# tangjiapeng/DiffuScene

Measured on AMD Instinct MI355X. Metric: denoiser steps/sec (train + 1000-step sample) at B=256, N=80 objects, higher is better.
Workload: dtype f32 (operands split 3xbf16, 6 products, f32 accumulate); 1 GPU; uncond living/dining rooms (config/uncond/diffusion_livingrooms_instancond_lat32_v.yaml scaled to N=80), B=256 scenes per GPU, N=80, C=65, T=1000, mode=both; global_batch=256, parallelism=single

## Files before the change

diffuscene_amd/_lib.py:

```python
import ctypes as C
import os

_HERE = os.path.dirname(os.path.abspath(__file__))
LIB_PATH = os.path.join(_HERE, "libdiffuscene_hip.so")
if os.environ.get("DSC_HIP_LIB"):
    LIB_PATH = os.path.abspath(os.environ["DSC_HIP_LIB"])

ACT_NONE, ACT_GELU, ACT_SILU, ACT_LEAKY01 = 0, 1, 2, 3
SS_NONE, SS_PER_TOKEN, SS_PER_SCENE, SS_PER_SLOT, SS_BY_INDEX = 0, 1, 2, 3, 4
MEAN_EPS, MEAN_X0, MEAN_V = 0, 1, 2
TILE_GN_80_W8, TILE_GN_80_W4, TILE_160x256, TILE_160x128_W4 = 1, 2, 5, 8
TILE_WAVE_GN, TILE_WAVE_DENSE, TILE_WAVE_GN_64 = 10, 11, 12
F32_TILE_160x256, F32_TILE_160x128, F32_TILE_128x128, F32_TILE_96x128, F32_TILE_64x64 = 0, 1, 2, 3, 4
DSC_PLANES_NONE = -100
GEMM_ROW_INVARIANT = 1
WS_MAX = 64
MAX_TOKENS_PER_SCENE = 160
STATS_MAX_OBJECTS, STATS_ONE_WAVE_MAX = 160, 32

_ERR = {-1: "DSC_EINVAL (bad shape / null pointer)", -2: "DSC_EALIGN (16-byte alignment required)",
        -3: "DSC_ERANGE (size outside kernel limits)"}

c_f32p = C.c_void_p
c_i64p = C.c_void_p
# ... 115 lines not shown
    "dsc_knn_cov_f32": (C.c_int, [c_f32p, C.c_int64, C.c_void_p, C.c_int32, C.c_int32, c_f32p, C.c_int64, C.c_void_p]),
    "dsc_gather_max_f32": (C.c_int, [c_f32p, C.c_int64, C.c_void_p, C.c_int32, C.c_int32, C.c_int32, c_f32p, C.c_int64,
                                     C.c_void_p, C.c_void_p]),
    "dsc_gather_max_bwd_f32": (C.c_int, [c_f32p, C.c_int64, C.c_void_p, C.c_void_p, C.c_int32, C.c_int32, C.c_int32, c_f32p,
                                         C.c_int64, C.c_void_p]),
    "dsc_bn_workspace_floats": (C.c_int64, [C.c_int64, C.c_int32]),
    "dsc_batchnorm_fwd_f32": (C.c_int, [c_f32p, C.c_int64, c_f32p, c_f32p, C.c_int64, C.c_int32, C.c_float, C.c_float,
                                        C.c_int32, c_f32p, c_f32p, c_f32p, c_f32p, c_f32p, c_f32p, c_f32p, C.c_int64,
                                        C.c_void_p]),
    "dsc_batchnorm_eval_f32": (C.c_int, [c_f32p, C.c_int64, c_f32p, c_f32p, c_f32p, c_f32p, C.c_int64, C.c_int32, C.c_int32,
                                         c_f32p, C.c_void_p]),
    "dsc_batchnorm_bwd_f32": (C.c_int, [c_f32p, c_f32p, c_f32p, c_f32p, c_f32p, C.c_int64, C.c_int32, C.c_int32, c_f32p,
                                        c_f32p, c_f32p, c_f32p, C.c_int64, C.c_void_p]),
    "dsc_rowmax_f32": (C.c_int, [c_f32p, C.c_int64, C.c_int32, C.c_int32, C.c_int32, c_f32p, C.c_void_p, C.c_void_p]),
    "dsc_rowmax_bwd_f32": (C.c_int, [c_f32p, C.c_void_p, C.c_int32, C.c_int32, C.c_int32, c_f32p, C.c_void_p]),
    "dsc_point_affine_f32": (C.c_int, [c_f32p, C.c_int64, C.c_int32, c_f32p, C.c_int64, c_f32p, C.c_int32, C.c_int32,
                                       C.c_int32, C.c_int32, c_f32p, C.c_void_p]),
    "dsc_point_affine_bwd_f32": (C.c_int, [c_f32p, c_f32p, C.c_int64, C.c_int32, c_f32p, C.c_int64, C.c_int32, C.c_int32,
                                           C.c_int32, C.c_int32, c_f32p, C.c_int64, c_f32p, C.c_int64, c_f32p, c_f32p,
                                           C.c_int64, C.c_void_p]),
    "dsc_postfilter_compact_f32": (C.c_int, [c_f32p, C.c_int32, C.c_int32, C.c_int32, C.c_int32, C.c_int32, C.c_int32, c_f32p,
                                             C.c_void_p, C.c_void_p]),
    "dsc_gemm_tn_f32": (C.c_int, [c_f32p, C.c_int64, C.c_int32, c_f32p, C.c_int64, C.c_int32, c_f32p, C.c_int64, c_f32p,
                                  C.c_int64, c_f32p, C.c_int32, C.c_int32, C.c_int32, c_f32p, C.c_int64, C.c_void_p]),
    "dsc_gemm_tn_workspace_floats": (C.c_int64, [C.c_int32, C.c_int32, C.c_int32]),
    "dsc_gemm_tn_grouped_f32": (C.c_int, [C.c_void_p, C.c_int32, C.c_int32, C.c_int32, c_f32p, C.c_int64, C.c_int64,
                                          C.c_void_p]),
    "dsc_gemm_tn_grouped_split_f32": (C.c_int, [C.c_void_p, C.c_int32, C.c_int32, C.c_void_p, C.c_int32, C.c_int32, c_f32p, C.c_int64,
                                                C.c_int64, C.c_int32, C.c_void_p]),
    "dsc_set_tn_split_form": (C.c_int, [C.c_int32]),
    "dsc_get_tn_split_form": (C.c_int, []),
    "dsc_colsum_f32": (C.c_int, [c_f32p, C.c_int64, C.c_int32, C.c_int32, c_f32p, c_f32p, C.c_int64, C.c_void_p]),
    "dsc_colsum_grouped_f32": (C.c_int, [C.c_void_p, C.c_int32, C.c_int32, C.c_void_p]),
    "dsc_gn_silu_bwd_f32": (C.c_int, [c_f32p, C.c_int64, c_f32p, C.c_int64, c_f32p, c_f32p, c_f32p, C.c_int64, C.c_int32,
                                      c_f32p, C.c_int64, c_f32p, c_f32p, c_f32p, C.c_int64, c_f32p, C.c_int64, C.c_int32,
                                      C.c_int32, C.c_int32, C.c_float, C.c_void_p]),
    "dsc_weight_standardize_bwd_f32": (C.c_int, [C.POINTER(WsBwdItem), C.c_int32, C.c_float, C.c_void_p]),
    "dsc_layernorm_bwd_f32": (C.c_int, [c_f32p, C.c_int64, c_f32p, c_f32p, C.c_int64, c_f32p, C.c_int64, c_f32p, C.c_int64, c_f32p,
                                        C.c_int32, C.c_int32, C.c_int32, C.c_float, C.c_void_p]),
    "dsc_linear_attention_bwd_f32": (C.c_int, [c_f32p, C.c_int64] * 7 + [C.c_int32, C.c_int32, C.c_int32, C.c_float,
                                                                          C.c_void_p]),
    "dsc_attention_bwd_f32": (C.c_int, [c_f32p, C.c_int64] * 7 + [C.c_int32, C.c_int32, C.c_float, C.c_void_p]),
    "dsc_retrieve_nearest_f32": (C.c_int, [c_f32p, C.c_void_p, C.c_void_p, c_f32p, C.c_void_p, C.c_void_p, C.c_int32,
                                           C.c_int32, C.c_int32, C.c_void_p, c_f32p, C.c_void_p]),
    "dsc_box_bounds_f32": (C.c_int, [c_f32p, c_f32p, c_f32p, C.c_void_p, C.c_int32, C.c_int32, c_f32p, C.c_void_p]),
    "dsc_scene_stats_f32": (C.c_int, [c_f32p, c_f32p, C.c_void_p, C.c_void_p, C.c_int32, C.c_int32, C.c_int32, C.c_int32,
                                      C.c_void_p, C.c_void_p, C.c_void_p, C.c_void_p, C.c_void_p, C.c_void_p, c_f32p, C.c_void_p]),
    "dsc_encode_scene_batch_f32": (C.c_int, [c_i64p, c_f32p, c_f32p, c_f32p, c_f32p, c_f32p, C.c_int32, C.c_int32, c_i64p,
                                             C.c_void_p, C.c_void_p, C.c_void_p, C.c_int32, C.POINTER(C.c_double), c_f32p,
                                             C.c_int64, c_i64p, C.c_int32, C.c_int32, C.c_void_p]),
    "dsc_chamfer3d_forward_f32": (C.c_int, [c_f32p, c_f32p, c_f32p, c_f32p, C.c_void_p, C.c_void_p, C.c_int32, C.c_int32,
                                            C.c_int32, C.c_void_p]),
    "dsc_chamfer3d_backward_f32": (C.c_int, [c_f32p, c_f32p, c_f32p, c_f32p, C.c_void_p, C.c_void_p, c_f32p, c_f32p,
                                             C.c_int32, C.c_int32, C.c_int32, C.c_void_p]),
    "dsc_grad_sumsq_f32": (C.c_int, [C.c_void_p, C.c_int32, C.c_void_p, C.c_void_p]),
    "dsc_clip_coef_f32": (C.c_int, [C.c_void_p, C.c_int32, C.c_float, c_f32p, c_f32p, C.c_void_p]),
    "dsc_adam_step_f32": (C.c_int, [C.c_void_p, C.c_int32, C.c_float, C.c_float, C.c_float, C.c_float, C.c_float, C.c_float,
                                    c_f32p, C.c_void_p]),
    "dsc_adam_ema_step_f32": (C.c_int, [C.c_void_p, C.c_void_p, C.c_int32, C.c_float, C.c_float, C.c_float, C.c_float, C.c_float,
                                        C.c_float, c_f32p, C.c_float, C.c_void_p]),
    "dsc_ema_update_f32": (C.c_int, [C.c_void_p, C.c_void_p, C.c_int32, C.c_float, C.c_void_p]),
    "dsc_ema_swap_f32": (C.c_int, [C.c_void_p, C.c_void_p, C.c_int32, C.c_void_p]),
    "dsc_ddpm_loss_f32": (C.c_int, [c_f32p, c_f32p, c_f32p, c_i64p, c_f32p, c_f32p, c_f32p, c_f32p, C.POINTER(C.c_float),
                                    c_f32p, c_f32p, c_f32p] + [C.c_int32] * 12 + [C.c_float, C.c_int32, C.c_void_p]),
    "dsc_copy2d_f32": (C.c_int, [c_f32p, C.c_int64, c_f32p, C.c_int64, C.c_int32, C.c_int32, C.c_void_p]),
    "dsc_add2d_f32": (C.c_int, [c_f32p, C.c_int64, c_f32p, C.c_int64, C.c_int32, C.c_int32, C.c_void_p]),
# ... 45 lines not shown
    "dsc_avgpool_rows_bwd_f32": (C.c_int, [c_f32p, c_f32p] + [C.c_int32] * 3 + [C.c_void_p]),
}

_lib = None


class HipLibraryMissing(RuntimeError):
    pass


def load():
    global _lib
    if _lib is not None:
        return _lib
    if not os.path.exists(LIB_PATH):
        raise HipLibraryMissing(
            "%s not found: build it with `python __graft_entry__.py` (hipcc --offload-arch=gfx950). "
            "diffuscene_amd has no CPU or PyTorch fallback." % LIB_PATH)
    import torch
    lib = C.CDLL(LIB_PATH)
    for name, (res, args) in SIGNATURES.items():
        try:
            fn = getattr(lib, name)
        except AttributeError as e:
            raise HipLibraryMissing("symbol %s missing from %s" % (name, LIB_PATH)) from e
        fn.restype = res
        fn.argtypes = args
    if lib.dsc_get_gemm_arithmetic() < 0:
        raise ValueError("DSC_GEMM=%r: must be 'split' (default) or 'f32'" % os.environ.get("DSC_GEMM"))
    if lib.dsc_get_tn_split_form() < 0:
        raise ValueError("DSC_TN_FORM=%r: must be '2' (default), '1' or '0'" % os.environ.get("DSC_TN_FORM"))
    if lib.dsc_get_split_wave() < 0:
        raise ValueError("DSC_WAVE=%r: must be '1' / 'auto' (default) or '0'" % os.environ.get("DSC_WAVE"))
    _lib = lib
    return lib


def split_enabled():
    return load().dsc_get_gemm_arithmetic() == 1


def gemm_mode():
    lib = load()
    if lib.dsc_get_gemm_arithmetic() != 1:
        return 0
    return (2 if lib.dsc_get_split_wave() == 1 else 1) + 10 * lib.dsc_get_tn_split_form()


def set_split_wave(on):
    prev = load().dsc_get_split_wave() == 1
    check(load().dsc_set_split_wave(1 if on else 0), "dsc_set_split_wave")
    return prev


def set_gemm_arithmetic(name):
    if name not in ("split", "f32"):
        raise ValueError("gemm arithmetic must be 'split' or 'f32', got %r" % (name,))
    prev = "split" if split_enabled() else "f32"
    check(load().dsc_set_gemm_arithmetic(1 if name == "split" else 0), "dsc_set_gemm_arithmetic")
    return prev


def device_error_count(reset=False):
    n = load().dsc_device_error_count(1 if reset else 0)
    if n < 0:
        raise RuntimeError("dsc_device_error_count failed (HIP error)")
    return int(n)


def check_indices(where):
    if os.environ.get("DSC_CHECK_INDICES", "0") == "1":
        n = device_error_count(reset=True)
        if n:
            raise IndexError("%s: %d out-of-range device timestep(s) were clamped into the schedule tables" % (where, n))


def check(rc, what):
    if rc != 0:
        raise RuntimeError("%s failed: %s" % (what, _ERR.get(rc, "hipError_t %d" % rc)))


def fn(name):
    return getattr(load(), name)
```

diffuscene_amd/csrc/train.hip:

```cpp
#define DSC_BAD_INDEX_COUNTER
#include "dsc_common.h"

namespace {

constexpr int TN_BK = 32;
constexpr int TN_LD = 132;

struct TnArgs {
    const float* a1; long lda1; int k1;
    const float* a2; long lda2; int k2;
    const float* dy; long ldd;
    float* out; long ldo;
    float* bias_out;
    long slab;
    long bias_slab;
    int m, n, kvalid;
    int chunk;
    int ktiles;
};

__device__ __forceinline__ void tn_block(const TnArgs& p, const int it, const int jt, const int split, float* As, float* Bs) {
    const int tid = threadIdx.x, lane = tid & 63, wave = tid >> 6;
    const int wi = wave >> 1, wj = wave & 1;
    const int l31 = lane & 31, half = lane >> 5;
    const int i0 = it * 128, j0 = jt * 128;
    const long m_begin = (long)split * p.chunk;
    const long m_end = (m_begin + p.chunk < p.m) ? m_begin + p.chunk : p.m;

    const float* ab;
    long lda;
    int ic;
    int kseg;
    if (i0 < p.k1) { ab = p.a1; lda = p.lda1; ic = i0; kseg = p.k1; }
// ... 523 lines not shown
            p.dss[(tok0 + j) * p.ld_dss + c] = du * gh;
            p.dss[(tok0 + j) * p.ld_dss + p.C + c] = du;
        }
        zc[j * 64] = xh;
        dc[j * 64] = dxh;
    }
    const float m1 = block_sum(S1, red) * inv_cnt;
    const float m2 = block_sum(S2, red) * inv_cnt;
    float Gz = 0.f;
    {
        float* op = p.dz + (tok0 + tq) * p.lddz + c;
        const long os = 4 * p.lddz;
        for (int j = tq; j < N; j += 4) {
            const float dzv = rs * (dc[j * 64] - m1 - zc[j * 64] * m2);
            *op = dzv;
            op += os;
            Gz += dzv;
        }
    }
    csum[0][tq][cl] = Gg; csum[1][tq][cl] = Gb; csum[2][tq][cl] = Gz; csum[3][tq][cl] = Gsc; csum[4][tq][cl] = Gsh;
    __syncthreads();
    if (tq == 0) {
        const long o = (long)b * p.pstride + c;
        p.dgamma_p[o] = (csum[0][0][cl] + csum[0][1][cl]) + (csum[0][2][cl] + csum[0][3][cl]);
        p.dbeta_p[o] = (csum[1][0][cl] + csum[1][1][cl]) + (csum[1][2][cl] + csum[1][3][cl]);
        p.dbias_p[o] = (csum[2][0][cl] + csum[2][1][cl]) + (csum[2][2][cl] + csum[2][3][cl]);
        if (p.dss && p.ss_mode == DSC_SS_PER_SCENE) {
            p.dss[(long)b * p.ld_dss + c] = (csum[3][0][cl] + csum[3][1][cl]) + (csum[3][2][cl] + csum[3][3][cl]);
            p.dss[(long)b * p.ld_dss + p.C + c] = (csum[4][0][cl] + csum[4][1][cl]) + (csum[4][2][cl] + csum[4][3][cl]);
        }
    }
}

template <int NIT>
__global__ __launch_bounds__(256) void gn_silu_bwd_reg_kernel(const GnBwdArgs p) {
    __shared__ float red[2][4];
    __shared__ float csum[5][4][64];
    const int b = blockIdx.x >> 3, g = blockIdx.x & 7;
    const int cq = threadIdx.x & 15, tr = threadIdx.x >> 4;
    const int wave = threadIdx.x >> 6;
    const int c = g * 64 + cq * 4;
    const int N = p.n_tok;
    const long tok0 = (long)b * N;
    const float inv_cnt = 1.0f / (64.0f * (float)N);
    int phase = 0;
    auto bsum = [&](float v) {
        v = wave_sum(v);
        float* r = red[phase & 1];
        ++phase;
        if ((threadIdx.x & 63) == 0) r[wave] = v;
        __syncthreads();
        return (r[0] + r[1]) + (r[2] + r[3]);
    };
    f32x4 zv[NIT], dv[NIT];
    float s = 0.f;
#pragma unroll
    for (int i = 0; i < NIT; ++i) {
        const int j = tr + 16 * i;
        const bool ok = j < N;
        const long row = tok0 + (ok ? j : 0);
        zv[i] = *reinterpret_cast<const f32x4*>(p.z + row * p.ldz + c);
        dv[i] = *reinterpret_cast<const f32x4*>(p.dy + row * p.ldy + c);
        if (!ok) { zv[i] = f32x4{0.f, 0.f, 0.f, 0.f}; dv[i] = zv[i]; }
        s += (zv[i][0] + zv[i][1]) + (zv[i][2] + zv[i][3]);
    }
    const float mu = bsum(s) * inv_cnt;
    s = 0.f;
#pragma unroll
    for (int i = 0; i < NIT; ++i)
        if (tr + 16 * i < N) {
#pragma unroll
            for (int e = 0; e < 4; ++e) { const float d = zv[i][e] - mu; s += d * d; }
        }
    const float rs = 1.0f / sqrtf(bsum(s) * inv_cnt + p.eps);
    const f32x4 ga = *reinterpret_cast<const f32x4*>(p.gamma + c);
    const f32x4 be = *reinterpret_cast<const f32x4*>(p.beta + c);
    const float* ssb = nullptr;
    long ss_step = 0;
    if (p.ss) {
        if (p.ss_mode == DSC_SS_PER_TOKEN) { ssb = p.ss + tok0 * p.ld_ss; ss_step = p.ld_ss; }
        else if (p.ss_mode == DSC_SS_PER_SCENE) { ssb = p.ss + (long)b * p.ld_ss; ss_step = 0; }
        else if (p.ss_mode == DSC_SS_PER_SLOT) { ssb = p.ss; ss_step = p.ld_ss; }
    }
    const bool dss_rows = p.dss && p.ss_mode != DSC_SS_PER_SCENE && ssb;
    float S1 = 0.f, S2 = 0.f;
    f32x4 Gg = {0.f, 0.f, 0.f, 0.f}, Gb = Gg, Gsc = Gg, Gsh = Gg, Gz = Gg;
#pragma unroll
    for (int i = 0; i < NIT; ++i) {
        const int j = tr + 16 * i;
        if (j < N) {
            f32x4 s1 = {1.f, 1.f, 1.f, 1.f}, sh = {0.f, 0.f, 0.f, 0.f};
            if (ssb) {
                const float* sr = ssb + (long)j * ss_step;
                const f32x4 a = *reinterpret_cast<const f32x4*>(sr + c);
                sh = *reinterpret_cast<const f32x4*>(sr + p.C + c);
#pragma unroll
                for (int e = 0; e < 4; ++e) s1[e] = 1.0f + a[e];
            }
            f32x4 xh, dxh, d_sc, d_sh;
#pragma unroll
            for (int e = 0; e < 4; ++e) {
                xh[e] = (zv[i][e] - mu) * rs;
                const float gh = ga[e] * xh[e] + be[e];
                const float u = gh * s1[e] + sh[e];
                const float sig = __builtin_amdgcn_rcpf(1.0f + __expf(-u));
                const float du = dv[i][e] * (sig * (1.0f + u * (1.0f - sig)));
                const float dgh = du * s1[e];
                dxh[e] = dgh * ga[e];
                S1 += dxh[e]; S2 += dxh[e] * xh[e];
                Gg[e] += dgh * xh[e]; Gb[e] += dgh; Gsc[e] += du * gh; Gsh[e] += du;
                d_sc[e] = du * gh; d_sh[e] = du;
            }
            if (dss_rows) {
                *reinterpret_cast<f32x4*>(p.dss + (tok0 + j) * p.ld_dss + c) = d_sc;
                *reinterpret_cast<f32x4*>(p.dss + (tok0 + j) * p.ld_dss + p.C + c) = d_sh;
            }
            zv[i] = xh;
            dv[i] = dxh;
        }
    }
    const float m1 = bsum(S1) * inv_cnt;
    const float m2 = bsum(S2) * inv_cnt;
#pragma unroll
    for (int i = 0; i < NIT; ++i) {
        const int j = tr + 16 * i;
        if (j < N) {
            f32x4 dzv;
#pragma unroll
            for (int e = 0; e < 4; ++e) { dzv[e] = rs * (dv[i][e] - m1 - zv[i][e] * m2); Gz[e] += dzv[e]; }
            *reinterpret_cast<f32x4*>(p.dz + (tok0 + j) * p.lddz + c) = dzv;
        }
    }
    auto fold = [&](f32x4 v, int slot) {
#pragma unroll
        for (int e = 0; e < 4; ++e) {
            float t = v[e];
            t += __shfl_xor(t, 16, 64);
            t += __shfl_xor(t, 32, 64);
            if ((threadIdx.x & 63) < 16) csum[slot][wave][cq * 4 + e] = t;
        }
    };
    fold(Gg, 0); fold(Gb, 1); fold(Gz, 2); fold(Gsc, 3); fold(Gsh, 4);
    __syncthreads();
    if (threadIdx.x < 64) {
        const int cl = threadIdx.x;
        const long o = (long)b * p.pstride + g * 64 + cl;
        p.dgamma_p[o] = (csum[0][0][cl] + csum[0][1][cl]) + (csum[0][2][cl] + csum[0][3][cl]);
        p.dbeta_p[o] = (csum[1][0][cl] + csum[1][1][cl]) + (csum[1][2][cl] + csum[1][3][cl]);
        p.dbias_p[o] = (csum[2][0][cl] + csum[2][1][cl]) + (csum[2][2][cl] + csum[2][3][cl]);
        if (p.dss && p.ss_mode == DSC_SS_PER_SCENE) {
            p.dss[(long)b * p.ld_dss + g * 64 + cl] = (csum[3][0][cl] + csum[3][1][cl]) + (csum[3][2][cl] + csum[3][3][cl]);
            p.dss[(long)b * p.ld_dss + p.C + g * 64 + cl] = (csum[4][0][cl] + csum[4][1][cl]) + (csum[4][2][cl] + csum[4][3][cl]);
        }
    }
}

struct WsBwdItem { const float* w; const float* dwh; float* dw; int rows; int cols; };
struct WsBwdBatch { WsBwdItem it[DSC_WS_MAX]; };

__global__ __launch_bounds__(256) void ws_bwd_kernel(const WsBwdBatch bch, const float eps) {
    __shared__ float red[4];
    const WsBwdItem it = bch.it[blockIdx.y];
    const int row = blockIdx.x;
    if (row >= it.rows) return;
    const float* w = it.w + (long)row * it.cols;
    const float* g = it.dwh + (long)row * it.cols;
    float* o = it.dw + (long)row * it.cols;
    constexpr int MAXE = 8;
    float v[MAXE], gv[MAXE];
    float s = 0.f;
#pragma unroll
    for (int i = 0; i < MAXE; ++i) {
        const int c = threadIdx.x + 256 * i;
        v[i] = (c < it.cols) ? w[c] : 0.f;
        gv[i] = (c < it.cols) ? g[c] : 0.f;
        s += v[i];
    }
    const float inv = 1.0f / (float)it.cols;
    const float mean = block_sum(s, red) * inv;
    float s2 = 0.f;
#pragma unroll
    for (int i = 0; i < MAXE; ++i) {
        const int c = threadIdx.x + 256 * i;
        const float d = (c < it.cols) ? v[i] - mean : 0.f;
        s2 += d * d;
// ... 641 lines not shown
                              int64_t workspace_floats, dsc_stream_t stream) {
    if (!x || !out || m < 1 || n < 1) return DSC_EINVAL;
    int splits = (m + 255) / 256;
    if (splits > 64) splits = 64;
    const int chunk = (m + splits - 1) / splits;
    splits = (m + chunk - 1) / chunk;
    hipStream_t s = static_cast<hipStream_t>(stream);
    if (splits == 1) {
        DSC_CLEAR_STALE_ERROR();
        hipLaunchKernelGGL(colsum_kernel, dim3((n + 63) / 64, 1), dim3(256), 0, s, x, (long)ldx, m, n, chunk, out);
        DSC_LAUNCH_CHECK();
        return 0;
    }
    if (!workspace || workspace_floats < (int64_t)splits * n) return DSC_EINVAL;
    DSC_CLEAR_STALE_ERROR();
    hipLaunchKernelGGL(colsum_kernel, dim3((n + 63) / 64, splits), dim3(256), 0, s, x, (long)ldx, m, n, chunk, workspace);
    DSC_LAUNCH_CHECK();
    DSC_CLEAR_STALE_ERROR();
    hipLaunchKernelGGL(reduce_slabs_kernel, dim3((n + 255) / 256), dim3(256), 0, s, workspace, (long)n, splits, out, (long)n);
    DSC_LAUNCH_CHECK();
    return 0;
}

extern "C" int dsc_colsum_grouped_f32(const dsc_colsum_item* items_dev, int32_t count, int32_t max_n, dsc_stream_t stream) {
    if (!items_dev || count < 1 || max_n < 1) return DSC_EINVAL;
    static_assert(sizeof(dsc_colsum_item) == sizeof(ColsumItem), "dsc_colsum_item layout");
    DSC_CLEAR_STALE_ERROR();
    hipLaunchKernelGGL(colsum_grouped_kernel, dim3((max_n + 63) / 64, count), dim3(256), 0, static_cast<hipStream_t>(stream),
                       reinterpret_cast<const ColsumItem*>(items_dev));
    DSC_LAUNCH_CHECK();
    return 0;
}

extern "C" int dsc_gn_silu_bwd_f32(const float* z, int64_t ldz, const float* dy, int64_t ldy, const float* gamma,
                                   const float* beta, const float* scale_shift, int64_t ld_ss, int32_t ss_mode,
                                   float* dz, int64_t lddz, float* dgamma_p, float* dbeta_p, float* dbias_p,
                                   int64_t partial_stride, float* dss, int64_t ld_dss, int32_t scenes,
                                   int32_t tokens_per_scene, int32_t channels, float eps, dsc_stream_t stream) {
    if (!z || !dy || !gamma || !beta || !dz || !dgamma_p || !dbeta_p || !dbias_p) return DSC_EINVAL;
    if (scenes < 1 || tokens_per_scene < 1 || channels != 512) return DSC_ERANGE;
    if (ss_mode != DSC_SS_NONE && !scale_shift) return DSC_EINVAL;
    GnBwdArgs p{z, (long)ldz, dy, (long)ldy, gamma, beta, ss_mode != DSC_SS_NONE ? scale_shift : nullptr, (long)ld_ss,
                ss_mode, dz, (long)lddz, dgamma_p, dbeta_p, dbias_p, (long)partial_stride, dss, (long)ld_dss, tokens_per_scene,
                channels, eps};
    if (tokens_per_scene > 160) return DSC_ERANGE;
    const size_t lds = (size_t)2 * tokens_per_scene * 64 * sizeof(float);
    DSC_CLEAR_STALE_ERROR();
    const bool v4 = ((ldz | ldy | lddz) & 3) == 0 && dsc_aligned16(z) && dsc_aligned16(dy) && dsc_aligned16(dz) &&
                    dsc_aligned16(gamma) && dsc_aligned16(beta) &&
                    (!p.ss || (dsc_aligned16(p.ss) && (ld_ss & 3) == 0)) &&
                    (!dss || (dsc_aligned16(dss) && (ld_dss & 3) == 0));
    if (lds > 48 * 1024) {
        static bool raised = false;
        if (!raised) {
            hipError_t e = hipFuncSetAttribute(reinterpret_cast<const void*>(gn_silu_bwd_kernel),
                                               hipFuncAttributeMaxDynamicSharedMemorySize, 96 * 1024);
            if (e != hipSuccess) return (int)e;
            raised = true;
        }
    }
    hipStream_t hs = static_cast<hipStream_t>(stream);
    if (v4 && tokens_per_scene <= 32)
        hipLaunchKernelGGL(gn_silu_bwd_reg_kernel<2>, dim3(scenes * 8), dim3(256), 0, hs, p);
    else if (v4 && tokens_per_scene <= 80)
        hipLaunchKernelGGL(gn_silu_bwd_reg_kernel<5>, dim3(scenes * 8), dim3(256), 0, hs, p);
    else if (v4)
        hipLaunchKernelGGL(gn_silu_bwd_reg_kernel<10>, dim3(scenes * 8), dim3(256), 0, hs, p);
    else
        hipLaunchKernelGGL(gn_silu_bwd_kernel, dim3(scenes * 8), dim3(256), lds, static_cast<hipStream_t>(stream), p);
    DSC_LAUNCH_CHECK();
    return 0;
}

extern "C" int dsc_weight_standardize_bwd_f32(const dsc_ws_bwd_item* items, int32_t count, float eps, dsc_stream_t stream) {
    if (!items || count < 1 || count > DSC_WS_MAX) return DSC_EINVAL;
    WsBwdBatch b;
    int maxrows = 0;
    for (int i = 0; i < count; ++i) {
        if (!items[i].w || !items[i].dw_std || !items[i].dw || items[i].rows < 1 || items[i].cols < 1) return DSC_EINVAL;
        if (items[i].cols > 2048) return DSC_ERANGE;
        b.it[i] = WsBwdItem{items[i].w, items[i].dw_std, items[i].dw, items[i].rows, items[i].cols};
        if (items[i].rows > maxrows) maxrows = items[i].rows;
    }
    DSC_CLEAR_STALE_ERROR();
    hipLaunchKernelGGL(ws_bwd_kernel, dim3(maxrows, count), dim3(256), 0, static_cast<hipStream_t>(stream), b, eps);
    DSC_LAUNCH_CHECK();
    return 0;
}

extern "C" int dsc_layernorm_bwd_f32(const float* x, int64_t ldx, const float* g, const float* dy, int64_t ldy, float* dx,
                                     int64_t lddx, const float* addend, int64_t ldadd, float* dg_partial, int32_t partial_rows,
                                     int32_t m, int32_t d, float eps, dsc_stream_t stream) {
    if (!x || !g || !dy || !dx || !dg_partial || m < 1 || partial_rows < 1) return DSC_EINVAL;
    if (d != 512) return DSC_ERANGE;
    if (!dsc_aligned16(x) || !dsc_aligned16(g) || !dsc_aligned16(dy) || !dsc_aligned16(dx) || (ldx & 3) || (ldy & 3) ||
        (lddx & 3) || (addend && (!dsc_aligned16(addend) || (ldadd & 3)))) return DSC_EALIGN;
    DSC_CLEAR_STALE_ERROR();
    hipLaunchKernelGGL(layernorm_bwd_kernel, dim3(partial_rows), dim3(256), 0, static_cast<hipStream_t>(stream),
                       x, (long)ldx, g, dy, (long)ldy, dx, (long)lddx, addend, (long)ldadd, dg_partial, m, eps);
    DSC_LAUNCH_CHECK();
// ... 392 lines not shown
```

include/diffuscene_hip.h:

```cpp
#ifndef DIFFUSCENE_HIP_H
#define DIFFUSCENE_HIP_H

#include <stdint.h>

#ifdef __cplusplus
extern "C" {
#endif

typedef void* dsc_stream_t;

#define DSC_EINVAL   (-1)
#define DSC_EALIGN   (-2)
#define DSC_ERANGE   (-3)

#define DSC_ACT_NONE 0
#define DSC_ACT_GELU 1
#define DSC_ACT_SILU 2
#define DSC_ACT_LEAKY01 3

#define DSC_SS_NONE      0
#define DSC_SS_PER_TOKEN 1
#define DSC_SS_PER_SCENE 2
#define DSC_SS_PER_SLOT  3
#define DSC_SS_BY_INDEX  4
// ... 256 lines not shown
int64_t dsc_gemm_tn_workspace_floats(int32_t m, int32_t n, int32_t k);

typedef struct dsc_tn_group {
    const float* a1; int64_t lda1; int32_t k1;
    const float* a2; int64_t lda2; int32_t k2;
    const float* dy; int64_t ldd;
    float* out; int64_t ldo;
    float* dbias;
    int32_t m, n, kvalid;
    int32_t tile0;
    int64_t ws_offset;
    int32_t tile0s;
} dsc_tn_group;
int dsc_gemm_tn_grouped_f32(const dsc_tn_group* groups_dev, int32_t count, int32_t total_tiles, int32_t splits,
                            float* workspace, int64_t workspace_floats, int64_t workspace_needed, dsc_stream_t stream);
int dsc_gemm_tn_grouped_split_f32(const dsc_tn_group* groups_dev, int32_t count, int32_t total_tiles, const int32_t* block_map_dev,
                                  int32_t blocks, int32_t splits, float* workspace, int64_t workspace_floats, int64_t workspace_needed,
                                  int32_t tile_k, dsc_stream_t stream);

int dsc_set_tn_split_form(int32_t form);
int dsc_get_tn_split_form(void);

int dsc_colsum_f32(const float* x, int64_t ldx, int32_t m, int32_t n, float* out, float* workspace,
                   int64_t workspace_floats, dsc_stream_t stream);

typedef struct dsc_colsum_item { const float* x; int64_t ldx; int32_t m, n; float* out; } dsc_colsum_item;
int dsc_colsum_grouped_f32(const dsc_colsum_item* items_dev, int32_t count, int32_t max_n, dsc_stream_t stream);

int dsc_gn_silu_bwd_f32(const float* z, int64_t ldz, const float* dy, int64_t ldy, const float* gamma,
                        const float* beta, const float* scale_shift, int64_t ld_ss, int32_t ss_mode,
                        float* dz, int64_t lddz, float* dgamma_p, float* dbeta_p, float* dbias_p, int64_t partial_stride,
                        float* dss, int64_t ld_dss, int32_t scenes, int32_t tokens_per_scene, int32_t channels,
                        float eps, dsc_stream_t stream);

typedef struct dsc_ws_bwd_item { const float* w; const float* dw_std; float* dw; int32_t rows; int32_t cols; } dsc_ws_bwd_item;
int dsc_weight_standardize_bwd_f32(const dsc_ws_bwd_item* items, int32_t count, float eps, dsc_stream_t stream);

int dsc_layernorm_bwd_f32(const float* x, int64_t ldx, const float* g, const float* dy, int64_t ldy, float* dx,
                          int64_t lddx, const float* addend, int64_t ldadd, float* dg_partial, int32_t partial_rows, int32_t m,
                          int32_t d, float eps, dsc_stream_t stream);

int dsc_linear_attention_bwd_f32(const float* q, int64_t ldq, const float* k, int64_t ldk, const float* v, int64_t ldv,
                                 const float* dout, int64_t ldo, float* dq, int64_t lddq, float* dk, int64_t lddk,
                                 float* dv, int64_t lddv, int32_t scenes, int32_t nq, int32_t nk, float scale,
                                 dsc_stream_t stream);

int dsc_attention_bwd_f32(const float* q, int64_t ldq, const float* k, int64_t ldk, const float* v, int64_t ldv,
                          const float* dout, int64_t ldo, float* dq, int64_t lddq, float* dk, int64_t lddk,
                          float* dv, int64_t lddv, int32_t scenes, int32_t n, float scale, dsc_stream_t stream);

int dsc_ddpm_loss_f32(const float* target, const float* out, const float* x_t, const int64_t* t,
                      const float* loss_weight, const float* ca, const float* cb, const float* alphas_cumprod,
                      const float* bounds, float* losses, float* parts, float* dout, int32_t b, int32_t n, int32_t c,
                      int32_t translation_dim, int32_t size_dim, int32_t bbox_dim, int32_t class_dim,
                      int32_t objectness_dim, int32_t objfeat_dim, int32_t loss_separate, int32_t loss_iou,
                      int32_t mean_type, float grad_scale, int32_t num_timesteps, dsc_stream_t stream);

int dsc_copy2d_f32(float* dst, int64_t ldd, const float* src, int64_t lds, int32_t rows, int32_t cols, dsc_stream_t stream);
int dsc_add2d_f32(float* dst, int64_t ldd, const float* src, int64_t lds, int32_t rows, int32_t cols, dsc_stream_t stream);

int dsc_activation_bwd_f32(const float* x, const float* dy, float* dx, int64_t count, int32_t act, dsc_stream_t stream);

int dsc_transpose_f32(const float* in, int64_t ldi, float* out, int64_t ldo, int32_t rows, int32_t cols,
                      dsc_stream_t stream);
int dsc_transpose_batched_f32(const dsc_ws_item* items, int32_t count, dsc_stream_t stream);

// ... 97 lines not shown
```

Baseline: 59.83 steps/s.

## Make GroupNorm-SiLU backward persistent with software-pipelined prefetch of next cell

Converts the GroupNorm+SiLU backward register kernel into a persistent grid sized to resident occupancy. Each block loops over (scene, group) cells and prefetches the next cell's z and dy into a second register set while it reduces the current one. It also uses ds_swizzle for intra-wave reductions and 32-bit offset addressing, and hoists per-scene scale/shift loads out of the token loop. The aim is to hide global load latency and cut launch tail effects, at the cost of doubled register footprint and a new env/API switch.

Result: slower. 58.30 steps/s (-2.6%).

```diff
diff --git a/diffuscene_amd/_lib.py b/diffuscene_amd/_lib.py
--- a/diffuscene_amd/_lib.py
+++ b/diffuscene_amd/_lib.py
@@ -171,6 +171,9 @@
     "dsc_get_tn_split_form": (C.c_int, []),
     "dsc_colsum_f32": (C.c_int, [c_f32p, C.c_int64, C.c_int32, C.c_int32, c_f32p, c_f32p, C.c_int64, C.c_void_p]),
     "dsc_colsum_grouped_f32": (C.c_int, [C.c_void_p, C.c_int32, C.c_int32, C.c_void_p]),
+    "dsc_get_gn_bwd_form": (C.c_int, []),
+    "dsc_set_gn_bwd_form": (C.c_int, [C.c_int32]),
+    "dsc_set_gn_bwd_grid_cap": (C.c_int, [C.c_int32]),
     "dsc_gn_silu_bwd_f32": (C.c_int, [c_f32p, C.c_int64, c_f32p, C.c_int64, c_f32p, c_f32p, c_f32p, C.c_int64, C.c_int32,
                                       c_f32p, C.c_int64, c_f32p, c_f32p, c_f32p, C.c_int64, c_f32p, C.c_int64, C.c_int32,
                                       C.c_int32, C.c_int32, C.c_float, C.c_void_p]),
@@ -282,6 +285,8 @@
         raise ValueError("DSC_TN_FORM=%r: must be '2' (default), '1' or '0'" % os.environ.get("DSC_TN_FORM"))
     if lib.dsc_get_split_wave() < 0:
         raise ValueError("DSC_WAVE=%r: must be '1' / 'auto' (default) or '0'" % os.environ.get("DSC_WAVE"))
+    if lib.dsc_get_gn_bwd_form() < 0:
+        raise ValueError("DSC_GN_BWD=%r: must be '1' (default) or '0'" % os.environ.get("DSC_GN_BWD"))
     _lib = lib
     return lib
 
@@ -300,6 +305,13 @@
 def set_split_wave(on):
     prev = load().dsc_get_split_wave() == 1
     check(load().dsc_set_split_wave(1 if on else 0), "dsc_set_split_wave")
+    return prev
+
+
+def set_gn_bwd_form(form, grid_cap=0):
+    prev = load().dsc_get_gn_bwd_form()
+    check(load().dsc_set_gn_bwd_form(int(form)), "dsc_set_gn_bwd_form")
+    check(load().dsc_set_gn_bwd_grid_cap(int(grid_cap)), "dsc_set_gn_bwd_grid_cap")
     return prev
 
 
diff --git a/diffuscene_amd/csrc/train.hip b/diffuscene_amd/csrc/train.hip
--- a/diffuscene_amd/csrc/train.hip
+++ b/diffuscene_amd/csrc/train.hip
@@ -1,4 +1,8 @@
 #define DSC_BAD_INDEX_COUNTER
+#include <algorithm>
+#include <atomic>
+#include <cstdlib>
+#include <cstring>
 #include "dsc_common.h"
 
 namespace {
@@ -588,125 +592,182 @@
     }
 }
 
-template <int NIT>
-__global__ __launch_bounds__(256) void gn_silu_bwd_reg_kernel(const GnBwdArgs p) {
+template <int NIT, bool PIPE, bool SSROWS>
+__global__ __launch_bounds__(256, PIPE ? 3 : 1) void gn_silu_bwd_reg_kernel(const GnBwdArgs p, const int ncell) {
     __shared__ float red[2][4];
     __shared__ float csum[5][4][64];
-    const int b = blockIdx.x >> 3, g = blockIdx.x & 7;
     const int cq = threadIdx.x & 15, tr = threadIdx.x >> 4;
     const int wave = threadIdx.x >> 6;
-    const int c = g * 64 + cq * 4;
     const int N = p.n_tok;
-    const long tok0 = (long)b * N;
     const float inv_cnt = 1.0f / (64.0f * (float)N);
     int phase = 0;
+    auto lane_xor = [](float v, auto o) {
+        constexpr int O = decltype(o)::value;
+        if constexpr (PIPE && O < 32)
+            return __builtin_bit_cast(float, __builtin_amdgcn_ds_swizzle(__builtin_bit_cast(int, v), (O << 10) | 0x1f));
+        else
+            return __shfl_xor(v, O, 64);
+    };
     auto bsum = [&](float v) {
-        v = wave_sum(v);
+        dsc_static_for<6>([&](auto k) { v += lane_xor(v, std::integral_constant<int, (32 >> decltype(k)::value)>{}); });
         float* r = red[phase & 1];
         ++phase;
         if ((threadIdx.x & 63) == 0) r[wave] = v;
         __syncthreads();
         return (r[0] + r[1]) + (r[2] + r[3]);
     };
-    f32x4 zv[NIT], dv[NIT];
-    float s = 0.f;
-#pragma unroll
-    for (int i = 0; i < NIT; ++i) {
-        const int j = tr + 16 * i;
-        const bool ok = j < N;
-        const long row = tok0 + (ok ? j : 0);
-        zv[i] = *reinterpret_cast<const f32x4*>(p.z + row * p.ldz + c);
-        dv[i] = *reinterpret_cast<const f32x4*>(p.dy + row * p.ldy + c);
-        if (!ok) { zv[i] = f32x4{0.f, 0.f, 0.f, 0.f}; dv[i] = zv[i]; }
-        s += (zv[i][0] + zv[i][1]) + (zv[i][2] + zv[i][3]);
-    }
-    const float mu = bsum(s) * inv_cnt;
-    s = 0.f;
-#pragma unroll
-    for (int i = 0; i < NIT; ++i)
-        if (tr + 16 * i < N) {
-#pragma unroll
-            for (int e = 0; e < 4; ++e) { const float d = zv[i][e] - mu; s += d * d; }
-        }
-    const float rs = 1.0f / sqrtf(bsum(s) * inv_cnt + p.eps);
-    const f32x4 ga = *reinterpret_cast<const f32x4*>(p.gamma + c);
-    const f32x4 be = *reinterpret_cast<const f32x4*>(p.beta + c);
-    const float* ssb = nullptr;
-    long ss_step = 0;
-    if (p.ss) {
-        if (p.ss_mode == DSC_SS_PER_TOKEN) { ssb = p.ss + tok0 * p.ld_ss; ss_step = p.ld_ss; }
-        else if (p.ss_mode == DSC_SS_PER_SCENE) { ssb = p.ss + (long)b * p.ld_ss; ss_step = 0; }
-        else if (p.ss_mode == DSC_SS_PER_SLOT) { ssb = p.ss; ss_step = p.ld_ss; }
-    }
-    const bool dss_rows = p.dss && p.ss_mode != DSC_SS_PER_SCENE && ssb;
-    float S1 = 0.f, S2 = 0.f;
-    f32x4 Gg = {0.f, 0.f, 0.f, 0.f}, Gb = Gg, Gsc = Gg, Gsh = Gg, Gz = Gg;
-#pragma unroll
-    for (int i = 0; i < NIT; ++i) {
-        const int j = tr + 16 * i;
-        if (j < N) {
-            f32x4 s1 = {1.f, 1.f, 1.f, 1.f}, sh = {0.f, 0.f, 0.f, 0.f};
-            if (ssb) {
-                const float* sr = ssb + (long)j * ss_step;
-                const f32x4 a = *reinterpret_cast<const f32x4*>(sr + c);
-                sh = *reinterpret_cast<const f32x4*>(sr + p.C + c);
-#pragma unroll
-                for (int e = 0; e < 4; ++e) s1[e] = 1.0f + a[e];
-            }
-            f32x4 xh, dxh, d_sc, d_sh;
+    auto at = [&](auto* x, long ld, int b_, int g_, int i, bool clamp) {
+        int t = tr;
+        if constexpr (PIPE) asm volatile("" : "+v"(t));
+        int j = t + 16 * i;
+        if (clamp) j = j < N ? j : 0;
+        if constexpr (PIPE) {
+            const unsigned off = ((unsigned)j * (unsigned)ld + (unsigned)(cq * 4)) * 4u;
+            return (decltype(x))((char*)(x + ((long)b_ * N * ld + g_ * 64)) + off);
+        } else {
+            return x + ((long)b_ * N + j) * ld + (g_ * 64 + cq * 4);
+        }
+    };
+    auto fetch = [&](int cell_, const float* x, long ldx, f32x4 (&v)[NIT]) {
+#pragma unroll
+        for (int i = 0; i < NIT; ++i) {
+            v[i] = *reinterpret_cast<const f32x4*>(at(x, ldx, cell_ >> 3, cell_ & 7, i, true));
+        }
+    };
+    auto do_cell = [&](const int cell, f32x4 (&zv)[NIT], f32x4 (&dv)[NIT], f32x4 (&zn)[NIT], f32x4 (&dn)[NIT]) {
+        const int b = cell >> 3, g = cell & 7;
+        const int c = g * 64 + cq * 4;
+        const long tok0 = (long)b * N;
+        const f32x4 ga = *reinterpret_cast<const f32x4*>(p.gamma + c);
+        const f32x4 be = *reinterpret_cast<const f32x4*>(p.beta + c);
+        const float* ssb = nullptr;
+        long ss_step = 0;
+        if (p.ss) {
+            if (SSROWS && p.ss_mode == DSC_SS_PER_TOKEN) { ssb = p.ss + tok0 * p.ld_ss; ss_step = p.ld_ss; }
+            else if (p.ss_mode == DSC_SS_PER_SCENE) { ssb = p.ss + (long)b * p.ld_ss; ss_step = 0; }
+            else if (SSROWS && p.ss_mode == DSC_SS_PER_SLOT) { ssb = p.ss; ss_step = p.ld_ss; }
+        }
+        f32x4 s1c = {0.f, 0.f, 0.f, 0.f}, shc = s1c;
+        if (!SSROWS && ssb) {
+            s1c = *reinterpret_cast<const f32x4*>(ssb + c);
+            shc = *reinterpret_cast<const f32x4*>(ssb + p.C + c);
+        }
+        const int nxt = cell + (int)gridDim.x;
+        float s = 0.f;
+#pragma unroll
+        for (int i = 0; i < NIT; ++i) {
+            if (!(tr + 16 * i < N)) { zv[i] = f32x4{0.f, 0.f, 0.f, 0.f}; dv[i] = zv[i]; }
+            s += (zv[i][0] + zv[i][1]) + (zv[i][2] + zv[i][3]);
+        }
+        const float mu = bsum(s) * inv_cnt;
+        s = 0.f;
+#pragma unroll
+        for (int i = 0; i < NIT; ++i)
+            if (tr + 16 * i < N) {
+#pragma unroll
+                for (int e = 0; e < 4; ++e) { const float d = zv[i][e] - mu; s += d * d; }
+            }
+        const float rs = 1.0f / sqrtf(bsum(s) * inv_cnt + p.eps);
+        if constexpr (PIPE && !SSROWS) {
+            __builtin_amdgcn_s_waitcnt(0x0f70);
+            if (nxt < ncell) fetch(nxt, p.z, p.ldz, zn);
+        }
+#pragma unroll
+        for (int e = 0; e < 4; ++e) s1c[e] = 1.0f + s1c[e];
+        const bool dss_rows = SSROWS && p.dss && p.ss_mode != DSC_SS_PER_SCENE && ssb;
+        float S1 = 0.f, S2 = 0.f;
+        f32x4 Gg = {0.f, 0.f, 0.f, 0.f}, Gb = Gg, Gsc = Gg, Gsh = Gg, Gz = Gg;
+#pragma unroll
+        for (int i = 0; i < NIT; ++i) {
+            const int j = tr + 16 * i;
+            if (j < N) {
+                f32x4 s1 = s1c, sh = shc;
+                if (SSROWS && ssb) {
+                    const float* sr = ssb + (long)j * ss_step;
+                    const f32x4 a = *reinterpret_cast<const f32x4*>(sr + c);
+                    sh = *reinterpret_cast<const f32x4*>(sr + p.C + c);
+#pragma unroll
+                    for (int e = 0; e < 4; ++e) s1[e] = 1.0f + a[e];
+                }
+                f32x4 xh, dxh, d_sc, d_sh;
+#pragma unroll
+                for (int e = 0; e < 4; ++e) {
+                    xh[e] = (zv[i][e] - mu) * rs;
+                    const float gh = ga[e] * xh[e] + be[e];
+                    const float u = gh * s1[e] + sh[e];
+                    const float sig = __builtin_amdgcn_rcpf(1.0f + __expf(-u));
+                    const float du = dv[i][e] * (sig * (1.0f + u * (1.0f - sig)));
+                    const float dgh = du * s1[e];
+                    dxh[e] = dgh * ga[e];
+                    S1 += dxh[e]; S2 += dxh[e] * xh[e];
+                    Gg[e] += dgh * xh[e]; Gb[e] += dgh; Gsc[e] += du * gh; Gsh[e] += du;
+                    d_sc[e] = du * gh; d_sh[e] = du;
+                }
+                if (dss_rows) {
+                    float* const o = at(p.dss, p.ld_dss, b, g, i, false);
+                    *reinterpret_cast<f32x4*>(o) = d_sc;
+                    *reinterpret_cast<f32x4*>(o + p.C) = d_sh;
+                }
+                zv[i] = xh;
+                dv[i] = dxh;
+                if constexpr (PIPE) asm volatile("");
+            }
+        }
+        const float m1 = bsum(S1) * inv_cnt;
+        if constexpr (PIPE) {
+            if (nxt < ncell) {
+                if constexpr (SSROWS) fetch(nxt, p.z, p.ldz, zn);
+                fetch(nxt, p.dy, p.ldy, dn);
+            }
+        }
+        const float m2 = bsum(S2) * inv_cnt;
+#pragma unroll
+        for (int i = 0; i < NIT; ++i) {
+            const int j = tr + 16 * i;
+            if (j < N) {
+                f32x4 dzv;
+#pragma unroll
+                for (int e = 0; e < 4; ++e) { dzv[e] = rs * (dv[i][e] - m1 - zv[i][e] * m2); Gz[e] += dzv[e]; }
+                *reinterpret_cast<f32x4*>(at(p.dz, p.lddz, b, g, i, false)) = dzv;
+            }
+        }
+        auto fold = [&](f32x4 v, int slot) {
 #pragma unroll
             for (int e = 0; e < 4; ++e) {
-                xh[e] = (zv[i][e] - mu) * rs;
-                const float gh = ga[e] * xh[e] + be[e];
-                const float u = gh * s1[e] + sh[e];
-                const float sig = __builtin_amdgcn_rcpf(1.0f + __expf(-u));
-                const float du = dv[i][e] * (sig * (1.0f + u * (1.0f - sig)));
-                const float dgh = du * s1[e];
-                dxh[e] = dgh * ga[e];
-                S1 += dxh[e]; S2 += dxh[e] * xh[e];
-                Gg[e] += dgh * xh[e]; Gb[e] += dgh; Gsc[e] += du * gh; Gsh[e] += du;
-                d_sc[e] = du * gh; d_sh[e] = du;
-            }
-            if (dss_rows) {
-                *reinterpret_cast<f32x4*>(p.dss + (tok0 + j) * p.ld_dss + c) = d_sc;
-                *reinterpret_cast<f32x4*>(p.dss + (tok0 + j) * p.ld_dss + p.C + c) = d_sh;
-            }
-            zv[i] = xh;
-            dv[i] = dxh;
-        }
-    }
-    const float m1 = bsum(S1) * inv_cnt;
-    const float m2 = bsum(S2) * inv_cnt;
-#pragma unroll
-    for (int i = 0; i < NIT; ++i) {
-        const int j = tr + 16 * i;
-        if (j < N) {
-            f32x4 dzv;
-#pragma unroll
-            for (int e = 0; e < 4; ++e) { dzv[e] = rs * (dv[i][e] - m1 - zv[i][e] * m2); Gz[e] += dzv[e]; }
-            *reinterpret_cast<f32x4*>(p.dz + (tok0 + j) * p.lddz + c) = dzv;
-        }
-    }
-    auto fold = [&](f32x4 v, int slot) {
-#pragma unroll
-        for (int e = 0; e < 4; ++e) {
-            float t = v[e];
-            t += __shfl_xor(t, 16, 64);
-            t += __shfl_xor(t, 32, 64);
-            if ((threadIdx.x & 63) < 16) csum[slot][wave][cq * 4 + e] = t;
+                float t = v[e];
+                t += lane_xor(t, std::integral_constant<int, 16>{});
+                t += lane_xor(t, std::integral_constant<int, 32>{});
+                if ((threadIdx.x & 63) < 16) csum[slot][wave][cq * 4 + e] = t;
+            }
+        };
+        fold(Gg, 0); fold(Gb, 1); fold(Gz, 2); fold(Gsc, 3); fold(Gsh, 4);
+        __syncthreads();
+        if (threadIdx.x < 64) {
+            const int cl = threadIdx.x;
+            const long o = (long)b * p.pstride + g * 64 + cl;
+            p.dgamma_p[o] = (csum[0][0][cl] + csum[0][1][cl]) + (csum[0][2][cl] + csum[0][3][cl]);
+            p.dbeta_p[o] = (csum[1][0][cl] + csum[1][1][cl]) + (csum[1][2][cl] + csum[1][3][cl]);
+            p.dbias_p[o] = (csum[2][0][cl] + csum[2][1][cl]) + (csum[2][2][cl] + csum[2][3][cl]);
+            if (p.dss && p.ss_mode == DSC_SS_PER_SCENE) {
+                p.dss[(long)b * p.ld_dss + g * 64 + cl] = (csum[3][0][cl] + csum[3][1][cl]) + (csum[3][2][cl] + csum[3][3][cl]);
+                p.dss[(long)b * p.ld_dss + p.C + g * 64 + cl] = (csum[4][0][cl] + csum[4][1][cl]) + (csum[4][2][cl] + csum[4][3][cl]);
+            }
         }
     };
-    fold(Gg, 0); fold(Gb, 1); fold(Gz, 2); fold(Gsc, 3); fold(Gsh, 4);
-    __syncthreads();
-    if (threadIdx.x < 64) {
-        const int cl = threadIdx.x;
-        const long o = (long)b * p.pstride + g * 64 + cl;
-        p.dgamma_p[o] = (csum[0][0][cl] + csum[0][1][cl]) + (csum[0][2][cl] + csum[0][3][cl]);
-        p.dbeta_p[o] = (csum[1][0][cl] + csum[1][1][cl]) + (csum[1][2][cl] + csum[1][3][cl]);
-        p.dbias_p[o] = (csum[2][0][cl] + csum[2][1][cl]) + (csum[2][2][cl] + csum[2][3][cl]);
-        if (p.dss && p.ss_mode == DSC_SS_PER_SCENE) {
-            p.dss[(long)b * p.ld_dss + g * 64 + cl] = (csum[3][0][cl] + csum[3][1][cl]) + (csum[3][2][cl] + csum[3][3][cl]);
-            p.dss[(long)b * p.ld_dss + p.C + g * 64 + cl] = (csum[4][0][cl] + csum[4][1][cl]) + (csum[4][2][cl] + csum[4][3][cl]);
+    f32x4 za[NIT], da[NIT], zb[NIT], db[NIT];
+    int cell = blockIdx.x;
+    if (cell >= ncell) return;
+    fetch(cell, p.z, p.ldz, za);
+    fetch(cell, p.dy, p.ldy, da);
+    if constexpr (!PIPE) {
+        do_cell(cell, za, da, zb, db);
+    } else {
+        const int stride = (int)gridDim.x;
+        for (;;) {
+            do_cell(cell, za, da, zb, db);
+            if ((cell += stride) >= ncell) break;
+            do_cell(cell, zb, db, za, da);
+            if ((cell += stride) >= ncell) break;
         }
     }
 }
@@ -1414,6 +1475,53 @@
     return 0;
 }
 
+static std::atomic<int> g_gn_bwd_form{-1000};
+static std::atomic<int> g_gn_bwd_grid_cap{0};
+
+extern "C" int dsc_get_gn_bwd_form(void) {
+    int m = g_gn_bwd_form.load(std::memory_order_relaxed);
+    if (m == -1000) {
+        const char* e = getenv("DSC_GN_BWD");
+        m = (!e || !e[0] || !strcmp(e, "1")) ? 1 : !strcmp(e, "0") ? 0 : DSC_EINVAL;
+        g_gn_bwd_form.store(m, std::memory_order_relaxed);
+    }
+    return m;
+}
+
+extern "C" int dsc_set_gn_bwd_form(int32_t form) {
+    if (form != 0 && form != 1) return DSC_EINVAL;
+    g_gn_bwd_form.store(form, std::memory_order_relaxed);
+    return 0;
+}
+
+extern "C" int dsc_set_gn_bwd_grid_cap(int32_t max_blocks) {
+    if (max_blocks < 0) return DSC_EINVAL;
+    g_gn_bwd_grid_cap.store(max_blocks, std::memory_order_relaxed);
+    return 0;
+}
+
+static int gn_bwd_resident_blocks(int nit, bool rows) {
+    constexpr int MAXDEV = 64;
+    static std::atomic<int> cache[4][MAXDEV];
+    int dev = 0;
+    hipError_t e = hipGetDevice(&dev);
+    if (e != hipSuccess) return -(int)e;
+    std::atomic<int>* slot = (dev >= 0 && dev < MAXDEV) ? &cache[(nit == 2 ? 0 : 2) + (rows ? 1 : 0)][dev] : nullptr;
+    int n = slot ? slot->load(std::memory_order_relaxed) : 0;
+    if (n > 0) return n;
+    int per_cu = 0, cus = 0;
+    e = nit == 2 ? (rows ? hipOccupancyMaxActiveBlocksPerMultiprocessor(&per_cu, gn_silu_bwd_reg_kernel<2, true, true>, 256, 0)
+                         : hipOccupancyMaxActiveBlocksPerMultiprocessor(&per_cu, gn_silu_bwd_reg_kernel<2, true, false>, 256, 0))
+                 : (rows ? hipOccupancyMaxActiveBlocksPerMultiprocessor(&per_cu, gn_silu_bwd_reg_kernel<5, true, true>, 256, 0)
+                         : hipOccupancyMaxActiveBlocksPerMultiprocessor(&per_cu, gn_silu_bwd_reg_kernel<5, true, false>, 256, 0));
+    if (e != hipSuccess) return -(int)e;
+    e = hipDeviceGetAttribute(&cus, hipDeviceAttributeMultiprocessorCount, dev);
+    if (e != hipSuccess) return -(int)e;
+    n = (per_cu > 0 ? per_cu : 1) * (cus > 0 ? cus : 1);
+    if (slot) slot->store(n, std::memory_order_relaxed);
+    return n;
+}
+
 extern "C" int dsc_gn_silu_bwd_f32(const float* z, int64_t ldz, const float* dy, int64_t ldy, const float* gamma,
                                    const float* beta, const float* scale_shift, int64_t ld_ss, int32_t ss_mode,
                                    float* dz, int64_t lddz, float* dgamma_p, float* dbeta_p, float* dbias_p,
@@ -1442,12 +1550,30 @@
         }
     }
     hipStream_t hs = static_cast<hipStream_t>(stream);
-    if (v4 && tokens_per_scene <= 32)
-        hipLaunchKernelGGL(gn_silu_bwd_reg_kernel<2>, dim3(scenes * 8), dim3(256), 0, hs, p);
+    const int ncell = scenes * 8;
+    const int form = dsc_get_gn_bwd_form();
+    if (form < 0) return DSC_EINVAL;
+    const bool pipe = form == 1;
+    const int64_t ld_max = std::max(std::max(ldz, ldy), std::max(lddz, dss ? ld_dss : 0));
+    const int64_t ld_min = std::min(std::min(ldz, ldy), std::min(lddz, dss ? ld_dss : lddz));
+    if (v4 && tokens_per_scene <= 80 && pipe && ld_min >= 0 && ld_max < (int64_t(1) << 23)) {
+        const int nit = tokens_per_scene <= 32 ? 2 : 5;
+        const bool rows = p.ss && (ss_mode == DSC_SS_PER_TOKEN || ss_mode == DSC_SS_PER_SLOT);
+        int grid = gn_bwd_resident_blocks(nit, rows);
+        if (grid < 0) return -grid;
+        const int cap = g_gn_bwd_grid_cap.load(std::memory_order_relaxed);
+        if (cap > 0 && grid > cap) grid = cap;
+        if (grid > ncell) grid = ncell;
+        if (nit == 2 && rows) hipLaunchKernelGGL((gn_silu_bwd_reg_kernel<2, true, true>), dim3(grid), dim3(256), 0, hs, p, ncell);
+        else if (nit == 2) hipLaunchKernelGGL((gn_silu_bwd_reg_kernel<2, true, false>), dim3(grid), dim3(256), 0, hs, p, ncell);
+        else if (rows) hipLaunchKernelGGL((gn_silu_bwd_reg_kernel<5, true, true>), dim3(grid), dim3(256), 0, hs, p, ncell);
+        else hipLaunchKernelGGL((gn_silu_bwd_reg_kernel<5, true, false>), dim3(grid), dim3(256), 0, hs, p, ncell);
+    } else if (v4 && tokens_per_scene <= 32)
+        hipLaunchKernelGGL((gn_silu_bwd_reg_kernel<2, false, true>), dim3(ncell), dim3(256), 0, hs, p, ncell);
     else if (v4 && tokens_per_scene <= 80)
-        hipLaunchKernelGGL(gn_silu_bwd_reg_kernel<5>, dim3(scenes * 8), dim3(256), 0, hs, p);
+        hipLaunchKernelGGL((gn_silu_bwd_reg_kernel<5, false, true>), dim3(ncell), dim3(256), 0, hs, p, ncell);
     else if (v4)
-        hipLaunchKernelGGL(gn_silu_bwd_reg_kernel<10>, dim3(scenes * 8), dim3(256), 0, hs, p);
+        hipLaunchKernelGGL((gn_silu_bwd_reg_kernel<10, false, true>), dim3(ncell), dim3(256), 0, hs, p, ncell);
     else
         hipLaunchKernelGGL(gn_silu_bwd_kernel, dim3(scenes * 8), dim3(256), lds, static_cast<hipStream_t>(stream), p);
     DSC_LAUNCH_CHECK();
diff --git a/include/diffuscene_hip.h b/include/diffuscene_hip.h
--- a/include/diffuscene_hip.h
+++ b/include/diffuscene_hip.h
@@ -312,6 +312,10 @@
                         float* dz, int64_t lddz, float* dgamma_p, float* dbeta_p, float* dbias_p, int64_t partial_stride,
                         float* dss, int64_t ld_dss, int32_t scenes, int32_t tokens_per_scene, int32_t channels,
                         float eps, dsc_stream_t stream);
+
+int dsc_get_gn_bwd_form(void);
+int dsc_set_gn_bwd_form(int32_t form);
+int dsc_set_gn_bwd_grid_cap(int32_t max_blocks);
 
 typedef struct dsc_ws_bwd_item { const float* w; const float* dw_std; float* dw; int32_t rows; int32_t cols; } dsc_ws_bwd_item;
 int dsc_weight_standardize_bwd_f32(const dsc_ws_bwd_item* items, int32_t count, float eps, dsc_stream_t stream);
```
